# succinctlabs/sp1

Measured on AMD Instinct MI355X. Metric: RISC-V cycles proved/sec (core shard prove): whole ShardProof of a full core shard of the reference's `fibonacci` guest, see config, higher is better.
Workload: dtype u32 (KoalaBear Montgomery words, exact integer arithmetic)

## Files before the change

sp1_amd/csrc/basefold.hip:

```cpp
#include "device_ctx.hpp"
#include "tensor_table.hpp"

namespace sp1hip {

struct ExtArg { uint32_t c[4]; };
__device__ __forceinline__ kb::Ext E(const ExtArg& a) { return kb::Ext{{a.c[0], a.c[1], a.c[2], a.c[3]}}; }

__global__ __launch_bounds__(256) void transpose_kernel(const uint32_t* __restrict__ in, uint32_t* __restrict__ out,
                                                        size_t in_rows, size_t in_cols) {
    __shared__ uint32_t tile[32][33];
    const size_t r0 = (size_t)blockIdx.y * 32, c0 = (size_t)blockIdx.x * 32;
    const int tx = threadIdx.x & 31, ty = threadIdx.x >> 5;
    for (int k = ty; k < 32; k += 8) {
        size_t r = r0 + k, c = c0 + tx;
        if (r < in_rows && c < in_cols) tile[k][tx] = in[r * in_cols + c];
    }
    __syncthreads();
    for (int k = ty; k < 32; k += 8) {
        size_t c = c0 + k, r = r0 + tx;
        if (r < in_rows && c < in_cols) out[c * in_rows + r] = tile[tx][k];
    }
}

template <bool TO>
__global__ void monty_convert_kernel(uint32_t* data, size_t n) {
    size_t i = (size_t)blockIdx.x * blockDim.x + threadIdx.x;
    const size_t step = (size_t)gridDim.x * blockDim.x;
    for (; i < n; i += step) data[i] = TO ? kb::to_monty(data[i]) : kb::from_monty(data[i]);
}

__global__ __launch_bounds__(256) void batch_kernel(const uint32_t* const* __restrict__ cols, uint32_t total_width,
                                                    uint32_t height, const uint32_t* __restrict__ coeffs,
                                                    uint32_t* __restrict__ out) {
    const uint32_t row = blockIdx.x * 256u + threadIdx.x;
    if (row >= height) return;
    kb::DotAcc acc;
    kb::dot_init(acc);
    for (uint32_t g = 0; g < total_width; g++) {
        const kb::Ext c{{coeffs[4 * g], coeffs[4 * g + 1], coeffs[4 * g + 2], coeffs[4 * g + 3]}};
        kb::dot_add(acc, c, gptr(cols[g])[row]);
    }
    const kb::Ext r = kb::dot_finish(acc);
#pragma unroll
    for (int k = 0; k < 4; k++) out[(size_t)k * height + row] = r.c[k];
}

struct FoldOpenDesc {
    const uint32_t* cw;
    const uint32_t* tree;
    uint32_t lg_c, vals_off, paths_off, pad;
};

__device__ __forceinline__ void fold_even_odd_at(const uint32_t* __restrict__ cw, int lg_n, const ExtArg& half_beta,
                                                 const uint32_t* __restrict__ tw_lo, const uint32_t* __restrict__ tw_hi,
                                                 uint32_t* __restrict__ out, uint32_t i) {
    const uint32_t n = 1u << lg_n, m = n >> 1;
    kb::Ext e0, e1;
#pragma unroll
    for (int k = 0; k < 4; k++) {
        const uint2 v = *reinterpret_cast<const uint2*>(cw + (size_t)k * n + 2 * (size_t)i);
        e0.c[k] = v.x;
        e1.c[k] = v.y;
    }
    const uint32_t br = kb::reverse_bits_len(2 * i, lg_n);
    const uint32_t ex = ((n - br) & (n - 1)) << (kb::TWO_ADICITY - lg_n);
    const uint32_t xinv = kb::mul(tw_hi[ex >> TW_LO_BITS], tw_lo[ex & (TW_LO - 1)]);
    const uint32_t inv2 = 0x00ffffffu;
    kb::Ext s = kb::ext_mul_base(kb::ext_add(e0, e1), inv2);
    kb::Ext d = kb::ext_mul_base(kb::ext_sub(e0, e1), xinv);
    kb::Ext r = kb::ext_add(s, kb::ext_mul(d, E(half_beta)));
#pragma unroll
    for (int k = 0; k < 4; k++) out[(size_t)k * m + i] = r.c[k];
}
__global__ __launch_bounds__(256) void fold_even_odd_kernel(const uint32_t* __restrict__ cw, int lg_n, ExtArg half_beta,
                                                            const uint32_t* __restrict__ tw_lo,
                                                            const uint32_t* __restrict__ tw_hi,
                                                            uint32_t* __restrict__ out) {
    const uint32_t i = blockIdx.x * 256u + threadIdx.x;
    if (i < (1u << (lg_n - 1))) fold_even_odd_at(cw, lg_n, half_beta, tw_lo, tw_hi, out, i);
}

__device__ __forceinline__ kb::Ext fold_mle_at(const uint32_t* __restrict__ mle, int lg_n, const ExtArg& beta,
                                               uint32_t* __restrict__ out, uint32_t i) {
    const uint32_t n = 1u << lg_n, m = n >> 1;
    kb::Ext a, b;
#pragma unroll
    for (int k = 0; k < 4; k++) {
        const uint2 v = *reinterpret_cast<const uint2*>(mle + (size_t)k * n + 2 * (size_t)i);
        a.c[k] = v.x;
        b.c[k] = v.y;
    }
    kb::Ext r = kb::ext_add(a, kb::ext_mul(b, E(beta)));
#pragma unroll
    for (int k = 0; k < 4; k++) out[(size_t)k * m + i] = r.c[k];
    return r;
}
__global__ __launch_bounds__(256) void fold_mle_kernel(const uint32_t* __restrict__ mle, int lg_n, ExtArg beta,
                                                       uint32_t* __restrict__ out) {
    const uint32_t i = blockIdx.x * 256u + threadIdx.x;
    if (i < (1u << (lg_n - 1))) (void)fold_mle_at(mle, lg_n, beta, out, i);
}

__device__ __forceinline__ void block_sum4(uint32_t (&v)[4], uint32_t* scratch);

__global__ __launch_bounds__(256) void fold_round_kernel(const uint32_t* __restrict__ cw, int lg_c, ExtArg half_beta,
                                                         const uint32_t* __restrict__ tw_lo, const uint32_t* __restrict__ tw_hi,
                                                         uint32_t* __restrict__ cw_out, uint32_t cw_blocks,
                                                         const uint32_t* __restrict__ mle, int lg_m, ExtArg beta,
                                                         uint32_t* __restrict__ mle_out, const uint32_t* __restrict__ eq_next,
                                                         uint32_t* __restrict__ partial) {
    __shared__ uint32_t scratch[16];
    if (blockIdx.x < cw_blocks) {
        const uint32_t i = blockIdx.x * 256u + threadIdx.x;
        if (i < (1u << (lg_c - 1))) fold_even_odd_at(cw, lg_c, half_beta, tw_lo, tw_hi, cw_out, i);
        return;
    }
    const uint32_t b = blockIdx.x - cw_blocks, i = b * 256u + threadIdx.x, m = 1u << (lg_m - 1);
    kb::Ext term = kb::ext_zero();
    if (i < m) {
        const kb::Ext r = fold_mle_at(mle, lg_m, beta, mle_out, i);
        if (eq_next && !(i & 1u)) {
            const uint32_t j = i >> 1, half = m >> 1;
            kb::Ext e;
#pragma unroll
            for (int k = 0; k < 4; k++) e.c[k] = eq_next[(size_t)k * half + j];
            term = kb::ext_mul(e, r);
        }
// ... 269 lines not shown
    hipLaunchKernelGGL(fixed_at_zero_partial_kernel, dim3(blocks), dim3(256), 0, s, d_mle, n, d_eq, (uint32_t*)part.p);
    SP1HIP_LAUNCH_CHECK();
    launch_sum_partials((const uint32_t*)part.p, blocks, 4u, d_out, s);
    SP1HIP_LAUNCH_CHECK();
    return SP1HIP_SUCCESS;
}

int fold_round_async(const uint32_t* d_cw, int lg_c, const uint32_t* d_mle, int lg_m, const kb::Ext& beta, uint32_t* d_cw_out,
                     uint32_t* d_mle_out, const uint32_t* d_eq_next, uint32_t* d_zero_val, uint32_t* d_partial, hipStream_t s) {
    SP1HIP_REQUIRE(lg_c >= 1 && lg_c <= kb::TWO_ADICITY && lg_m >= 1 && lg_m <= 30, "fold sizes out of range");
    const DeviceCtx* ctx;
    SP1HIP_TRY(get_device_ctx(&ctx));
    ExtArg hb, b;
    for (int k = 0; k < 4; k++) { hb.c[k] = kb::mul(beta.c[k], 0x00ffffffu); b.c[k] = beta.c[k]; }
    const uint32_t cw_blocks = ((1u << (lg_c - 1)) + 255) / 256, mle_blocks = ((1u << (lg_m - 1)) + 255) / 256;
    hipLaunchKernelGGL(fold_round_kernel, dim3(cw_blocks + mle_blocks), dim3(256), 0, s, d_cw, lg_c, hb, ctx->d_tw_lo, ctx->d_tw_hi,
                       d_cw_out, cw_blocks, d_mle, lg_m, b, d_mle_out, d_eq_next, d_partial);
    SP1HIP_LAUNCH_CHECK();
    if (d_eq_next) {
        launch_sum_partials(d_partial, mle_blocks, 4u, d_zero_val, s);
        SP1HIP_LAUNCH_CHECK();
    }
    return SP1HIP_SUCCESS;
}

int eq_prefix_tables_soa_async(const kb::Ext* h_point, int d, uint32_t* d_out, hipStream_t s) {
    SP1HIP_REQUIRE(d >= 0 && d <= kb::TWO_ADICITY + 6, "dim out of range");
    PointArg pt;
    for (int j = 0; j < d; j++)
        for (int k = 0; k < 4; k++) pt.c[j][k] = h_point[j].c[k];
    hipLaunchKernelGGL(eq_prefix_soa_kernel, dim3(((1u << d) + 255) / 256), dim3(256), 0, s, pt, d, d_out);
    SP1HIP_LAUNCH_CHECK();
    return SP1HIP_SUCCESS;
}
}

extern "C" {

int sp1hip_transpose_to_col_major(uint32_t* d_out, const uint32_t* d_in, size_t rows, size_t cols, sp1hip_stream_t stream) {
    if (rows == 0 || cols == 0) return SP1HIP_SUCCESS;
    SP1HIP_REQUIRE(d_out && d_in && d_out != d_in, "bad buffers");
    dim3 grid((unsigned)((cols + 31) / 32), (unsigned)((rows + 31) / 32));
    SP1HIP_REQUIRE(grid.y <= 65535u * 1024u, "too many rows");
    hipLaunchKernelGGL(transpose_kernel, grid, dim3(256), 0, S(stream), d_in, d_out, rows, cols);
    SP1HIP_LAUNCH_CHECK();
    return SP1HIP_SUCCESS;
}

int sp1hip_transpose_to_row_major(uint32_t* d_out, const uint32_t* d_in, size_t rows, size_t cols, sp1hip_stream_t stream) {
    if (rows == 0 || cols == 0) return SP1HIP_SUCCESS;
    SP1HIP_REQUIRE(d_out && d_in && d_out != d_in, "bad buffers");
    dim3 grid((unsigned)((rows + 31) / 32), (unsigned)((cols + 31) / 32));
    hipLaunchKernelGGL(transpose_kernel, grid, dim3(256), 0, S(stream), d_in, d_out, cols, rows);
    SP1HIP_LAUNCH_CHECK();
    return SP1HIP_SUCCESS;
}

static int monty_convert(uint32_t* d, size_t n, bool to, sp1hip_stream_t stream) {
    if (!n) return SP1HIP_SUCCESS;
    SP1HIP_REQUIRE(d, "null buffer");
    size_t blocks = (n + 255) / 256;
    if (blocks > 4096) blocks = 4096;
    if (to) hipLaunchKernelGGL(monty_convert_kernel<true>, dim3((unsigned)blocks), dim3(256), 0, S(stream), d, n);
    else hipLaunchKernelGGL(monty_convert_kernel<false>, dim3((unsigned)blocks), dim3(256), 0, S(stream), d, n);
    SP1HIP_LAUNCH_CHECK();
    return SP1HIP_SUCCESS;
}
int sp1hip_to_monty(uint32_t* d, size_t n, sp1hip_stream_t s) { return monty_convert(d, n, true, s); }
int sp1hip_from_monty(uint32_t* d, size_t n, sp1hip_stream_t s) { return monty_convert(d, n, false, s); }

int sp1hip_basefold_batch(const sp1hip_tensor_t* tensors, int n_tensors, int lg_height, const uint32_t* d_coeffs,
                          uint32_t* d_out, sp1hip_stream_t stream) {
    SP1HIP_REQUIRE(lg_height >= 0 && lg_height <= 30, "lg_height out of range");
    SP1HIP_REQUIRE(d_coeffs && d_out, "null buffer");
    TensorTable tab;
    uint32_t tw;
    SP1HIP_TRY(make_tensor_table(tensors, n_tensors, &tab, &tw));
    SP1HIP_REQUIRE(tw <= 65536, "more than 2^16 columns in one message (batch_kernel's unreduced accumulators hold 2^16 terms)");
    hipStream_t s = S(stream);
    const uint32_t height = 1u << lg_height;
    AsyncScratch cols;
    SP1HIP_TRY(cols.alloc((size_t)tw * sizeof(uint32_t*), s));
    SP1HIP_TRY(expand_columns_async(tab, tw, height, (const uint32_t**)cols.p, s));
    hipLaunchKernelGGL(batch_kernel, dim3((height + 255) / 256), dim3(256), 0, s, (const uint32_t* const*)cols.p, tw,
                       height, d_coeffs, d_out);
    SP1HIP_LAUNCH_CHECK();
    return SP1HIP_SUCCESS;
}

int sp1hip_fold_even_odd(const uint32_t* d_cw, int lg_n, sp1hip_ext_t beta, uint32_t* d_out, sp1hip_stream_t stream) {
    SP1HIP_REQUIRE(lg_n >= 1 && lg_n <= kb::TWO_ADICITY, "lg_n out of range");
    SP1HIP_REQUIRE(d_cw && d_out, "null buffer");
    const DeviceCtx* ctx;
    SP1HIP_TRY(get_device_ctx(&ctx));
    ExtArg hb;
    for (int k = 0; k < 4; k++) hb.c[k] = kb::mul(beta.c[k], 0x00ffffffu);
    const uint32_t m = 1u << (lg_n - 1);
    hipLaunchKernelGGL(fold_even_odd_kernel, dim3((m + 255) / 256), dim3(256), 0, S(stream), d_cw, lg_n, hb,
                       ctx->d_tw_lo, ctx->d_tw_hi, d_out);
    SP1HIP_LAUNCH_CHECK();
    return SP1HIP_SUCCESS;
}

int sp1hip_fold_mle(const uint32_t* d_mle, int lg_n, sp1hip_ext_t beta, uint32_t* d_out, sp1hip_stream_t stream) {
    SP1HIP_REQUIRE(lg_n >= 1 && lg_n <= 30, "lg_n out of range");
    SP1HIP_REQUIRE(d_mle && d_out, "null buffer");
    ExtArg b;
    for (int k = 0; k < 4; k++) b.c[k] = beta.c[k];
    const uint32_t m = 1u << (lg_n - 1);
    hipLaunchKernelGGL(fold_mle_kernel, dim3((m + 255) / 256), dim3(256), 0, S(stream), d_mle, lg_n, b, d_out);
    SP1HIP_LAUNCH_CHECK();
    return SP1HIP_SUCCESS;
}

int sp1hip_partial_lagrange(const sp1hip_ext_t* h_point, int dim, uint32_t* d_out, sp1hip_stream_t stream) {
    SP1HIP_REQUIRE(dim >= 0 && dim <= kb::TWO_ADICITY + 6, "dim out of range");
    SP1HIP_REQUIRE(d_out && (h_point || dim == 0), "null buffer");
    hipStream_t s = S(stream);
    PointArg pt;
    for (int j = 0; j < dim; j++)
        for (int k = 0; k < 4; k++) pt.c[j][k] = h_point[j].c[k];
    const int d_hi = dim / 2, d_lo = dim - d_hi;
    AsyncScratch small;
    SP1HIP_TRY(small.alloc((((size_t)1 << d_hi) + ((size_t)1 << d_lo)) * 16, s));
    uint32_t* hi = (uint32_t*)small.p;
    uint32_t* lo = hi + ((size_t)4 << d_hi);
    hipLaunchKernelGGL(eq_small_kernel, dim3(((1u << d_hi) + 255) / 256), dim3(256), 0, s, pt, 0, d_hi, hi);
    SP1HIP_LAUNCH_CHECK();
    hipLaunchKernelGGL(eq_small_kernel, dim3(((1u << d_lo) + 255) / 256), dim3(256), 0, s, pt, d_hi, d_lo, lo);
    SP1HIP_LAUNCH_CHECK();
    const uint32_t len = 1u << dim;
    hipLaunchKernelGGL(eq_outer_kernel, dim3((len + 255) / 256), dim3(256), 0, s, hi, lo, d_lo, len, d_out);
    SP1HIP_LAUNCH_CHECK();
    return SP1HIP_SUCCESS;
}

int sp1hip_mle_eval_columns(const sp1hip_tensor_t* tensors, int n_tensors, int lg_height, const uint32_t* d_eq,
                            uint32_t* d_evals, sp1hip_stream_t stream) {
    SP1HIP_REQUIRE(lg_height >= 0 && lg_height <= 30, "lg_height out of range");
    SP1HIP_REQUIRE(d_eq && d_evals, "null buffer");
    TensorTable tab;
    uint32_t tw;
    SP1HIP_TRY(make_tensor_table(tensors, n_tensors, &tab, &tw));
    if (tw == 0) return SP1HIP_SUCCESS;
    SP1HIP_REQUIRE(tw <= 65536, "more than 2^16 columns in one message (the unreduced accumulators hold 2^16 terms)");
    hipStream_t s = S(stream);
    const uint32_t height = 1u << lg_height;
    AsyncScratch cols, part;
    SP1HIP_TRY(cols.alloc((size_t)tw * sizeof(uint32_t*), s));
    SP1HIP_TRY(expand_columns_async(tab, tw, height, (const uint32_t**)cols.p, s));
    const uint32_t chunks = (height + EVAL_ROWS - 1) / EVAL_ROWS;
    SP1HIP_TRY(part.alloc((size_t)chunks * tw * 16, s));
    dim3 grid((tw + EVAL_COLS - 1) / EVAL_COLS, chunks);
    hipLaunchKernelGGL(eval_columns_partial_kernel, grid, dim3(256), 0, s, (const uint32_t* const*)cols.p, tw, height,
                       d_eq, (uint32_t*)part.p);
    SP1HIP_LAUNCH_CHECK();
    launch_sum_partials((const uint32_t*)part.p, chunks, tw * 4, d_evals, s);
    SP1HIP_LAUNCH_CHECK();
    return SP1HIP_SUCCESS;
}

int sp1hip_ext_fixed_at_zero(const uint32_t* d_mle, int lg_n, const uint32_t* d_eq, uint32_t* d_out,
                             sp1hip_stream_t stream) {
    SP1HIP_REQUIRE(lg_n >= 1 && lg_n <= 30, "lg_n out of range");
    SP1HIP_REQUIRE(d_mle && d_eq && d_out, "null buffer");
    return ext_fixed_at_zero_async(d_mle, lg_n, d_eq, d_out, S(stream));
}

// ... 2 lines not shown
```

sp1_amd/csrc/gkr.hip:

```cpp
#include <algorithm>
#include <array>
#include <chrono>
#include <cstring>
#include <memory>
#include <string>
#include <vector>

#include "device_ctx.hpp"
#include "host_par.hpp"

namespace sp1hip {
bool gkr_host_simd_available();
void gkr_host_round_sums(const uint32_t* tab, size_t stride, const uint32_t* eq, size_t eq_stride, size_t real_pairs, uint32_t out[6][4]);
void gkr_host_round_fold(const uint32_t* tab, uint32_t* out, size_t stride, size_t real_pairs, const uint32_t alpha[4]);
}
#include "round_sync.hpp"
#include "tensor_table.hpp"

namespace sp1hip {

void challenger_observe(sp1hip_challenger_t* ch, uint32_t x);
kb::Ext challenger_sample_ext(sp1hip_challenger_t* ch);
void challenger_restore(sp1hip_challenger_t* dst, const sp1hip_challenger_t* src);
void challenger_export(const sp1hip_challenger_t* ch, uint32_t* w34);
// ... 420 lines not shown
        out[6] = (j & 1u) == 0 ? a[2] : z; out[7] = (j & 1u) == 0 ? z : a[2];
        out[8] = j < 2 ? a[3] : z;
        out[9] = a[4];
    } else {
        out[0] = j == 0 ? a[0] : z; out[1] = j == 1 ? a[0] : z;
        out[2] = a[1];
        out[3] = a[2];
    }
}

struct FlatArgs { const uint16_t* index; uint32_t total_slots; };

template <int FV, int SV, bool FIRST, bool NBASE, bool FLAT>
__global__ __launch_bounds__(256) void gkr_pass(const PassDesc* __restrict__ descs, const Ext* __restrict__ eq_int,
                                                const Ext* __restrict__ T, const Ext* __restrict__ TL, Ext a0, Ext a1,
                                                uint32_t* __restrict__ partials, RoundSync rs, uint32_t seq, uint32_t K,
                                                uint32_t tile_size, FlatArgs fa) {
    static_assert(FV + SV > 0 && FV <= 2 && SV <= 2, "a pass folds and / or sums");
    constexpr int SVS = SV == 0 ? 1 : SV;
    GridAcc<SVS> g;
    grid_init<SVS>(g);
    const uint32_t j = threadIdx.x & ((1u << SV) - 1u);
    auto do_row = [&](const PassDesc& d, uint32_t ro, bool valid, const Ext& wi, bool use_wi) {
        const uint32_t rows_out = (d.rows_in + (1u << FV) - 1u) >> FV;
        Row row = padding_row();
        if (valid && ro < rows_out) {
            row = fold_row<FV, FIRST, NBASE>(d, ro, a0, a1);
            if (FV > 0) {
                const uint32_t rq = folded_pos(ro, rows_out);
                if (SV == 0 && rs.host_slot != nullptr) {
                    st_ext_host(d.dst[0], rq, row.n0); st_ext_host(d.dst[1], rq, row.d0); st_ext_host(d.dst[2], rq, row.n1); st_ext_host(d.dst[3], rq, row.d1);
                } else {
                    st_ext(d.dst[0], rq, row.n0); st_ext(d.dst[1], rq, row.d0); st_ext(d.dst[2], rq, row.n1); st_ext(d.dst[3], rq, row.d1);
                }
            }
        }
        if constexpr (SV > 0) {
            const uint32_t cells = (rows_out + (1u << SV) - 1u) >> SV;
            const uint32_t c = ro >> SV;
            Ext w = kb::ext_zero(), wl = kb::ext_zero();
            if (valid && c < cells) {
                w = ld_ext(T, c); wl = ld_ext(TL, c);
                if (use_wi) { w = kb::ext_mul(w, wi); wl = kb::ext_mul(wl, wi); }
            }
            grid_accumulate<SVS, FIRST && NBASE && FV == 0>(row, w, wl, j, g);
        }
    };
    Ext scale = kb::ext_one();
    if (FLAT) {
        const uint32_t p = blockIdx.x * 256 + threadIdx.x;
        const bool valid = p < fa.total_slots;
        const PassDesc d = descs[valid ? fa.index[p] : 0];
        const Ext wi = SV > 0 ? ld_ext(eq_int, d.eq_int_index) : kb::ext_one();
        do_row(d, p - d.tile0, valid, wi, true);
    } else {
        const PassDesc d = descs[find_desc(descs, K, blockIdx.x)];
        const uint32_t rows_out = (d.rows_in + (1u << FV) - 1u) >> FV;
        const uint32_t slots = ((rows_out + (1u << SV) - 1u) >> SV) << SV;
        const uint32_t k0 = (blockIdx.x - d.tile0) * tile_size, k1 = min(slots, k0 + tile_size);
        for (uint32_t base = k0; base < k1; base += 256) do_row(d, base + threadIdx.x, base + threadIdx.x < k1, scale, false);
        if (SV > 0) scale = ld_ext(eq_int, d.eq_int_index);
    }
    if constexpr (SV > 0) {
        Ext out[GridOut<SVS>::NS];
        grid_split<SVS>(g, j, scale, !FLAT, out);
        rs_finish<GridOut<SVS>::NS>(out, partials, blockIdx.x, gridDim.x, rs, seq);
    } else if (rs.host_slot != nullptr) {
        asm volatile("s_waitcnt vmcnt(0)" ::: "memory");
        __syncthreads();
        if (threadIdx.x == 0 && rs_ticket_is_last_acq_rel(rs.counter, blockIdx.x, gridDim.x)) rs_publish_seq(rs.host_slot, seq);
    }
}

struct OpenDesc { const uint32_t* cols; uint32_t rows, width, col0, out0; };
constexpr int OPEN_COLS = 4, OPEN_ROWS = 16384;
__global__ __launch_bounds__(256) void open_columns_kernel(const OpenDesc* __restrict__ descs, const uint32_t* __restrict__ eq,
                                                           uint32_t eq_len, uint32_t* __restrict__ partials, uint32_t total_cols) {
    const OpenDesc d = descs[blockIdx.x];
    const uint32_t r0 = blockIdx.y * OPEN_ROWS;
    if (r0 >= d.rows) return;
    kb::DotAcc acc[OPEN_COLS];
#pragma unroll
    for (int c = 0; c < OPEN_COLS; c++) kb::dot_init(acc[c]);
    for (uint32_t r = r0 + threadIdx.x; r < r0 + OPEN_ROWS && r < d.rows; r += 256) {
        const Ext e{{eq[r], eq[eq_len + r], eq[2 * (size_t)eq_len + r], eq[3 * (size_t)eq_len + r]}};
#pragma unroll
        for (int c = 0; c < OPEN_COLS; c++)
            if (d.col0 + c < d.width) kb::dot_add(acc[c], e, gptr(d.cols)[(size_t)(d.col0 + c) * d.rows + r]);
    }
    __shared__ uint32_t sm[4][4 * OPEN_COLS];
    const int lane = threadIdx.x & 63, wave = threadIdx.x >> 6;
#pragma unroll
    for (int c = 0; c < OPEN_COLS; c++) {
        const Ext v = kb::dot_finish(acc[c]);
#pragma unroll
        for (int k = 0; k < 4; k++) {
            const uint32_t w = wave_sum(v.c[k]);
            if (lane == 0) sm[wave][4 * c + k] = w;
        }
    }
    __syncthreads();
    if (threadIdx.x < 4 * OPEN_COLS) {
        const int c = threadIdx.x / 4;
        if (d.col0 + c < d.width) {
            uint32_t a = 0;
            for (int i = 0; i < 4; i++) a = kb::add(a, sm[i][threadIdx.x]);
            partials[((size_t)blockIdx.y * total_cols + d.out0 + c) * 4 + (threadIdx.x & 3)] = a;
        }
    }
}
__global__ __launch_bounds__(256) void open_sum_kernel(const uint32_t* __restrict__ partials, uint32_t n_chunks, uint32_t n_words, uint32_t* __restrict__ out) {
    __shared__ uint32_t sm[256];
    const uint32_t jl = threadIdx.x & 63u, cl = threadIdx.x >> 6, j = blockIdx.x * 64u + jl;
    uint32_t acc = 0;
    if (j < n_words)
        for (uint32_t c = cl; c < n_chunks; c += 4) acc = kb::add(acc, partials[(size_t)c * n_words + j]);
    sm[threadIdx.x] = acc;
    __syncthreads();
    if (cl == 0 && j < n_words) out[j] = kb::add(kb::add(sm[jl], sm[64 + jl]), kb::add(sm[128 + jl], sm[192 + jl]));
}

Ext operator+(const Ext& a, const Ext& b) { return kb::ext_add(a, b); }
Ext operator-(const Ext& a, const Ext& b) { return kb::ext_sub(a, b); }
Ext operator*(const Ext& a, const Ext& b) { return kb::ext_mul(a, b); }
Ext ext_c(uint32_t canonical) { return kb::ext_from_base(kb::to_monty(canonical)); }
int log2_ceil(uint64_t x) { int l = 0; while (((uint64_t)1 << l) < x) l++; return l; }

std::vector<Ext> partial_lagrange_host(const std::vector<Ext>& pt) {
    std::vector<Ext> ev{kb::ext_one()};
    for (const Ext& x : pt) {
        std::vector<Ext> nx(ev.size() * 2);
        for (size_t i = 0; i < ev.size(); i++) { const Ext pr = ev[i] * x; nx[2 * i] = ev[i] - pr; nx[2 * i + 1] = pr; }
        ev.swap(nx);
    }
    return ev;
}
Ext eval_mle_host(const std::vector<Ext>& vals, const std::vector<Ext>& pt) {
    const std::vector<Ext> eq = partial_lagrange_host(pt);
    Ext acc = kb::ext_zero();
    for (size_t i = 0; i < vals.size(); i++) acc = acc + eq[i] * vals[i];
    return acc;
}

using Poly4 = std::array<Ext, 4>;
Ext poly_eval(const Poly4& c, const Ext& x) { return ((c[3] * x + c[2]) * x + c[1]) * x + c[0]; }

Poly4 interpolate4(const Ext (&xs)[4], const Ext (&ys)[4]) {
    Poly4 res{kb::ext_zero(), kb::ext_zero(), kb::ext_zero(), kb::ext_zero()};
    Ext num[4][4], den[4];
    bool live[4];
    for (int i = 0; i < 4; i++) {
        live[i] = !kb::ext_eq(ys[i], kb::ext_zero());
        if (!live[i]) continue;
        den[i] = kb::ext_one();
        Ext cur[4] = {ys[i], kb::ext_zero(), kb::ext_zero(), kb::ext_zero()};
        int deg = 0;
        for (int j = 0; j < 4; j++) {
            if (j == i) continue;
            den[i] = den[i] * (xs[i] - xs[j]);
            Ext nxt[4] = {kb::ext_zero(), kb::ext_zero(), kb::ext_zero(), kb::ext_zero()};
            for (int k = 0; k <= deg; k++) { nxt[k + 1] = nxt[k + 1] + cur[k]; nxt[k] = nxt[k] - cur[k] * xs[j]; }
            deg++;
            for (int k = 0; k < 4; k++) cur[k] = nxt[k];
        }
        for (int k = 0; k < 4; k++) num[i][k] = cur[k];
    }
    Ext prefix[4], running = kb::ext_one();
    for (int i = 0; i < 4; i++) if (live[i]) { prefix[i] = running; running = running * den[i]; }
    Ext inv_all = kb::ext_inv(running);
    for (int i = 3; i >= 0; i--) {
        if (!live[i]) continue;
// ... 738 lines not shown
```

sp1_amd/csrc/jagged.hip:

```cpp
#include <cstring>
#include <memory>
#include <vector>

#include <algorithm>
#include <array>

#include "device_ctx.hpp"
#include "jagged_host.hpp"
#include "round_sync.hpp"
#include "stacked_data.hpp"
#include "tensor_table.hpp"

namespace sp1hip {

struct DeviceBuf : AsyncScratch {
    uint32_t* u32() const { return (uint32_t*)p; }
};

void challenger_observe(sp1hip_challenger_t* ch, uint32_t x);
kb::Ext challenger_sample_ext(sp1hip_challenger_t* ch);
void challenger_restore(sp1hip_challenger_t* dst, const sp1hip_challenger_t* src);

using Ext = kb::Ext;

// ... 933 lines not shown
        uint32_t g = T;
        for (uint32_t pfx : prefix) g |= pfx;
        rf = g ? __builtin_ctz(g) : 0;
        rf = std::min(rf, std::min(log_m - 2, max_log_row_count - 1));
        if (!factored_enabled) rf = 0;
        if (rf < 2) rf = 0;
    }
    bool j_materialised = rf == 0;
    if (rf == 0) {
        SP1HIP_TRY(tabs[1].alloc((size_t)std::max<uint32_t>(n1, 1) * 16, s));
        SP1HIP_TRY(tabs[3].alloc((size_t)std::max<uint32_t>((n1 + 1) / 2, 1) * 16, s));
    }
    DeviceBuf row_eq_lv[2], d_prefix_lv;
    const uint32_t* row_eq_cur = d_row_eq.u32();
    uint32_t row_len_cur = 1u << max_log_row_count;
    if (rf) {
        SP1HIP_TRY(row_eq_lv[0].alloc(((size_t)16) << (max_log_row_count - 1), s));
        SP1HIP_TRY(row_eq_lv[1].alloc(((size_t)16) << (max_log_row_count - 1), s));
        SP1HIP_TRY(d_prefix_lv.alloc(prefix.size() * 4 * (size_t)(rf + 1), s));
        std::vector<uint32_t> all_lv(prefix.size() * (size_t)(rf + 1));
        for (int lv = 0; lv <= rf; lv++)
            for (size_t c = 0; c < prefix.size(); c++) all_lv[(size_t)lv * prefix.size() + c] = prefix[c] >> lv;
        SP1HIP_TRY(sc.stage.upload(d_prefix_lv.p, all_lv.data(), all_lv.size() * 4));
    }
    auto level_J = [&](int lv, const Ext& a_prev, JgJ* out) -> int {
        uint32_t* dst = row_eq_lv[lv & 1].u32();
        hipLaunchKernelGGL(jg_fold_row_eq, dim3((row_len_cur / 2 + 255) / 256), dim3(256), 0, s, row_eq_cur, row_len_cur, a_prev, dst);
        SP1HIP_LAUNCH_CHECK();
        row_eq_cur = dst;
        row_len_cur >>= 1;
        uint32_t* d_pl = d_prefix_lv.u32() + (size_t)lv * prefix.size();
        *out = JgJ{d_pl, ncols, (const Ext*)d_col_eq.p, row_eq_cur, row_len_cur};
        return SP1HIP_SUCCESS;
    };
    std::vector<JgTab> tabs0;
    uint32_t n_tiles0 = 0, n_tiles1 = 0, n_tiles2 = 0;
    bool tables_mult4 = false;
    bool skip_level1 = false;
    std::vector<std::pair<uint64_t, uint64_t>> zero_tails;
    DeviceBuf d_tabs0, d_col_eq3;
    {
        uint32_t g = T;
        for (uint32_t pfx : prefix) g |= pfx;
        if ((g & 1u) == 0 && factored_enabled) {
            uint64_t seg_start = 0;
            uint32_t col = 0;
            for (int r = 0; r < n_rounds; r++) {
                const StackedCore* d = rounds[r];
                uint64_t off = 0;
                const size_t n_real = d->row_counts.size() - 2;
                for (size_t t = 0; t < d->row_counts.size(); t++) {
                    const uint32_t h = (uint32_t)d->row_counts[t], w = (uint32_t)d->column_counts[t];
                    if (t < n_real && h && w) {
                        for (uint32_t c_lo = 0; c_lo < w; c_lo += JG_COL_SLICE) {
                            const uint32_t wc = std::min(JG_COL_SLICE, w - c_lo);
                            const uint64_t o = off + (uint64_t)c_lo * h;
                            tabs0.push_back(JgTab{(const uint32_t*)d->d_dense + o, h, col + c_lo, wc, n_tiles0, (uint32_t)(seg_start + o), n_tiles1, n_tiles2});
                            n_tiles0 += (h / 2 + JG_TAB_PAIRS - 1) / JG_TAB_PAIRS;
                            n_tiles1 += ((h + 3) / 4 + JG_TAB_PAIRS - 1) / JG_TAB_PAIRS;
                            n_tiles2 += ((h + 7) / 8 + JG_TAB_PAIRS - 1) / JG_TAB_PAIRS;
                        }
                    }
                    if (t == n_real) zero_tails.push_back({seg_start + off, seg_start + d->padded});
                    off += (uint64_t)h * w;
                    col += w;
                }
                seg_start += d->padded;
            }
            if (!tabs0.empty()) {
                SP1HIP_TRY(upload(d_tabs0, tabs0.data(), tabs0.size() * sizeof(JgTab), s, sc.stage));
                tables_mult4 = (g & 3u) == 0;
                skip_level1 = (g & 7u) == 0 && rf >= 2 && log_m >= 4;
                std::vector<Ext> col_eq3(col_eq.size());
                for (size_t c = 0; c < col_eq.size(); c++)
                    for (int q = 0; q < 4; q++) col_eq3[c].c[q] = kb::add(kb::dbl(col_eq[c].c[q]), col_eq[c].c[q]);
                SP1HIP_TRY(upload(d_col_eq3, col_eq3.data(), col_eq3.size() * 16, s, sc.stage));
            }
        }
    }
    SP1HIP_TRY(tabs[0].alloc((size_t)std::max<uint32_t>(skip_level1 ? (T + 7) / 8 : n1, 1) * 16, s));
    SP1HIP_TRY(tabs[2].alloc((size_t)std::max<uint32_t>((n1 + 1) / 2, 1) * 16, s));
    uint32_t n_live = T;
    int cur = 0;
    jg_t[1] = std::chrono::steady_clock::now();
    const bool lookahead01 = skip_level1 && !tabs0.empty() && log_m >= 2 && env_flag("SP1HIP_JAGGED_LOOKAHEAD", true);
    for (int round = 0; round < log_m; round++) {
        uint32_t nb;
        if (round == 0 && lookahead01) {
            {
                ScopedTimer t("jagged_round0_sum", s);
                nb = Scratch::blocks_for((uint64_t)n_tiles1 * 256);
                hipLaunchKernelGGL(jg_round01_tables, dim3(nb), dim3(256), 0, s, (const JgTab*)d_tabs0.p, (uint32_t)tabs0.size(), n_tiles1, J,
                                   sc.tail());
                SP1HIP_LAUNCH_CHECK();
            }
            Ext S[8];
            SP1HIP_TRY(sc.finish8(S));
            const Ext y0 = S[0] + S[1], h0 = S[2] + S[3];
            poly = interpolate(y0, h0, claim - y0);
            sumcheck.polys.push_back(poly);
            alpha = observe_and_sample(ch, poly);
            alphas.push_back(alpha);
            claim = poly_eval(poly, alpha);
            {
                JgJ J1;
                SP1HIP_TRY(level_J(1, alpha, &J1));
            }
            const Ext a0 = alpha;
            const Ext c0 = S[0], c2 = (S[0] + S[4]) + (S[0] + S[4]) - S[2], c1 = S[4] - c0 - c2;
            const Ext d0 = S[5], d2 = S[7], d1 = S[6] - d0 - d2;
            const Ext y1 = c0 + (c1 + c2 * a0) * a0, h1 = d0 + (d1 + d2 * a0) * a0;
            poly = interpolate(y1, h1, claim - y1);
            sumcheck.polys.push_back(poly);
            alpha = observe_and_sample(ch, poly);
            alphas.push_back(alpha);
            claim = poly_eval(poly, alpha);
            n_live = (n_live + 1) / 2;
            cur = 0;
            round = 1;
            continue;
        }
        if (round == 0) {
            ScopedTimer t("jagged_round0_sum", s);
            if (!tabs0.empty()) {
                nb = Scratch::blocks_for((uint64_t)n_tiles0 * 256);
                hipLaunchKernelGGL(jg_round0_tables, dim3(nb), dim3(256), 0, s, (const JgTab*)d_tabs0.p, (uint32_t)tabs0.size(), n_tiles0, J,
                                   sc.tail());
            } else {
                nb = Scratch::blocks_for((T / 2 + JG_ITERS - 1) / JG_ITERS);
                hipLaunchKernelGGL(jg_round0_sum, dim3(nb), dim3(256), 0, s, segs, J, T / 2, sc.tail());
            }
        } else if (round == 1) {
            ScopedTimer t("jagged_fold0_sum", s);
            const uint32_t n_out = (n_live + 1) / 2;
            nb = Scratch::blocks_for(((n_out + 1) / 2 + JG_ITERS - 1) / JG_ITERS);
            if (rf) {
                JgJ J1;
                SP1HIP_TRY(level_J(1, alpha, &J1));
                if (skip_level1) {
                    nb = Scratch::blocks_for((uint64_t)n_tiles1 * 256);
                    hipLaunchKernelGGL((jg_fold_tables<1, false>), dim3(nb), dim3(256), 0, s, (const JgTab*)d_tabs0.p, (uint32_t)tabs0.size(),
                                       n_tiles1, J1, (const Ext*)d_col_eq3.p, alpha, alpha, (Ext*)nullptr, sc.tail());
                } else if (tables_mult4) {
                    for (auto& z : zero_tails)
                        if (z.second > z.first) SP1HIP_HIP(hipMemsetAsync((Ext*)tabs[0].p + z.first / 2, 0, (size_t)((z.second - z.first) / 2) * 16, s));
                    nb = Scratch::blocks_for((uint64_t)n_tiles1 * 256);
                    hipLaunchKernelGGL((jg_fold_tables<1, true>), dim3(nb), dim3(256), 0, s, (const JgTab*)d_tabs0.p, (uint32_t)tabs0.size(),
                                       n_tiles1, J1, (const Ext*)d_col_eq3.p, alpha, alpha, (Ext*)tabs[0].p, sc.tail());
                } else {
                    hipLaunchKernelGGL(jg_fold0_sum<false>, dim3(nb), dim3(256), 0, s, segs, J, alpha, n_out, (Ext*)tabs[0].p, (Ext*)nullptr,
                                       sc.tail());
                }
            } else {
                hipLaunchKernelGGL(jg_fold0_sum<true>, dim3(nb), dim3(256), 0, s, segs, J, alpha, n_out, (Ext*)tabs[0].p, (Ext*)tabs[1].p,
                                   sc.tail());
            }
            n_live = n_out;
            cur = 0;
        } else {
            ScopedTimer t("jagged_fold_sum", s);
            const uint32_t n_out = (n_live + 1) / 2;
            const int nxt = cur ^ 2;
            if (round == 2 && skip_level1) {
                JgJ Jl;
                SP1HIP_TRY(level_J(2, alpha, &Jl));
                for (auto& z : zero_tails)
                    if (z.second > z.first) SP1HIP_HIP(hipMemsetAsync((Ext*)tabs[nxt].p + z.first / 4, 0, (size_t)((z.second - z.first) / 4) * 16, s));
                nb = Scratch::blocks_for((uint64_t)n_tiles2 * 256);
                hipLaunchKernelGGL((jg_fold_tables<2, true>), dim3(nb), dim3(256), 0, s, (const JgTab*)d_tabs0.p, (uint32_t)tabs0.size(),
                                   n_tiles2, Jl, (const Ext*)d_col_eq3.p, alphas[0], alpha, (Ext*)tabs[nxt].p, sc.tail());
            } else if (round <= rf) {
                JgJ Jl;
                SP1HIP_TRY(level_J(round, alpha, &Jl));
                nb = Scratch::blocks_for(((n_out + 1) / 2 + JG_ITERS - 1) / JG_ITERS);
                hipLaunchKernelGGL(jg_foldf_sum, dim3(nb), dim3(256), 0, s, (const Ext*)tabs[cur].p, n_live, Jl, alpha, n_out,
                                   (Ext*)tabs[nxt].p, sc.tail());
            } else {
                nb = Scratch::blocks_for((n_out + 1) / 2);
                if (!j_materialised) {
                    const JgJ Jp{d_prefix_lv.u32() + (size_t)(round - 1) * prefix.size(), ncols, (const Ext*)d_col_eq.p, row_eq_cur, row_len_cur};
                    SP1HIP_TRY(tabs[cur + 1].alloc((size_t)std::max<uint32_t>((n_out + 1) / 2, 1) * 16, s));
                    SP1HIP_TRY(tabs[nxt + 1].alloc((size_t)std::max<uint32_t>(n_out, 1) * 16, s));
                    j_materialised = true;
                    hipLaunchKernelGGL(jg_fold_sum_fj, dim3(nb), dim3(256), 0, s, (const Ext*)tabs[cur].p, Jp, n_live, alpha, n_out,
                                       (Ext*)tabs[nxt].p, (Ext*)tabs[nxt + 1].p, sc.tail());
                } else {
                    hipLaunchKernelGGL(jg_fold_sum, dim3(nb), dim3(256), 0, s, (const Ext*)tabs[cur].p, (const Ext*)tabs[cur + 1].p, n_live,
                                       alpha, n_out, (Ext*)tabs[nxt].p, (Ext*)tabs[nxt + 1].p, sc.tail());
                }
            }
            n_live = n_out;
            cur = nxt;
        }
        SP1HIP_LAUNCH_CHECK();
        Ext y0, h4;
        SP1HIP_TRY(sc.finish(nb, &y0, &h4));
        poly = interpolate(y0, h4, claim - y0);
        sumcheck.polys.push_back(poly);
        alpha = observe_and_sample(ch, poly);
        alphas.push_back(alpha);
        claim = poly_eval(poly, alpha);
    }
    sumcheck.point.assign(alphas.rbegin(), alphas.rend());
    sumcheck.eval = claim;
    if (log_m == 0) {
        SP1HIP_REQUIRE(false, "degenerate dense area");
    } else if (log_m == 1) {
        uint32_t hq[2];
        SP1HIP_TRY(sc.mb.fetch(rounds[0]->d_dense, 2, hq));
        q_eval = kb::ext_from_base(hq[0]) + kb::ext_mul_base(alpha, kb::sub(hq[1], hq[0]));
    } else {
        Ext hq[2] = {kb::ext_zero(), kb::ext_zero()}, hj[2] = {kb::ext_zero(), kb::ext_zero()};
        SP1HIP_TRY(sc.mb.fetch(tabs[cur].p, (size_t)n_live * 4, hq));
        SP1HIP_TRY(sc.mb.fetch(tabs[cur + 1].p, (size_t)n_live * 4, hj));
        q_eval = hq[0] + alpha * (hq[1] - hq[0]);
        j_eval = hj[0] + alpha * (hj[1] - hj[0]);
    }
    (void)j_eval;
    const std::vector<Ext>& final_point = sumcheck.point;

    jg_t[2] = std::chrono::steady_clock::now();
    marks.next("jagged_eval");
    Sumcheck jagged_eval;
    SP1HIP_TRY(jagged_eval_prove(prefix, log_m, z_row, z_col, final_point, ch, sc, &jagged_eval));
    jg_t[3] = std::chrono::steady_clock::now();
    marks.next("stacked_basefold_open");

    for (int k = 0; k < 4; k++) ch.observe(q_eval.c[k]);
    const std::vector<Ext> stack_point(final_point.end() - lsh, final_point.end());
    DeviceBuf d_eq, d_evals;
    SP1HIP_TRY(d_eq.alloc(((size_t)16) << lsh, s));
    SP1HIP_TRY(sp1hip_partial_lagrange(reinterpret_cast<const sp1hip_ext_t*>(stack_point.data()), lsh, d_eq.u32(), stream));
    std::vector<std::vector<Ext>> batch_evals(n_rounds);
    std::vector<Ext> flat_claims;
    SP1HIP_TRY(d_evals.alloc((size_t)(*std::max_element(round_widths.begin(), round_widths.end())) * 16, s));
    for (int r = 0; r < n_rounds; r++) {
        const uint32_t w = round_widths[r];
        batch_evals[r].resize(w);
        ScopedTimer t("jagged_batch_evals", s);
        SP1HIP_TRY(sp1hip_mle_eval_columns(rounds[r]->batches.data(), (int)rounds[r]->batches.size(), lsh, d_eq.u32(), d_evals.u32(), stream));
        SP1HIP_TRY(sc.mb.fetch(d_evals.p, (size_t)w * 4, batch_evals[r].data()));
        flat_claims.insert(flat_claims.end(), batch_evals[r].begin(), batch_evals[r].end());
    }
    for (auto& e : flat_claims) for (int k = 0; k < 4; k++) ch.observe(e.c[k]);
    jg_t[4] = std::chrono::steady_clock::now();
    size_t bf_len = need;
    SP1HIP_TRY(be.open(reinterpret_cast<const sp1hip_ext_t*>(stack_point.data()), lsh,
                       reinterpret_cast<const sp1hip_ext_t*>(flat_claims.data()), flat_claims.size(), config, h_proof, &bf_len, stream));

    jg_t[5] = std::chrono::steady_clock::now();
    Bytes w;
    w.p = h_proof;
    w.cap = need;
    w.n = bf_len;
    w.u64(n_rounds);
    for (auto& ev : batch_evals) { w.u64(ev.size()); for (auto& e : ev) w.ext(e); w.u64(1); w.u64(ev.size()); }
    sumcheck.write(w);
    jagged_eval.write(w);
    w.u64(n_rounds);
    for (int r = 0; r < n_rounds; r++) {
        w.u64(rounds[r]->row_counts.size());
        for (size_t t = 0; t < rounds[r]->row_counts.size(); t++) { w.u64(rounds[r]->row_counts[t]); w.u64(rounds[r]->column_counts[t]); }
    }
    w.u64(n_rounds);
    for (int r = 0; r < n_rounds; r++) {
        uint8_t c[64];
        be.write_commitment(r, c);
        w.raw(c, be.commitment_bytes());
    }
    w.ext(q_eval);
    w.u64(max_log_row_count);
    w.u64(log_m);
    if (w.overflow || w.n != need) {
        set_error("internal error: jagged proof size %zu != expected %zu", w.n, need);
        return SP1HIP_ERROR_RUNTIME;
    }
    *proof_len = w.n;
    be.accept();
    if (jg_timing) {
        jg_t[6] = std::chrono::steady_clock::now();
        const auto ms = [&](int a, int b) { return std::chrono::duration<double, std::milli>(jg_t[b] - jg_t[a]).count(); };
        fprintf(stderr, "[sp1hip jagged] set-up %.3f ms | %d sumcheck rounds %.3f | jagged-eval %.3f | column evaluations %.3f | BaseFold %.3f | proof bytes %.3f\n",
                ms(0, 1), log_m, ms(1, 2), ms(2, 3), ms(3, 4), ms(4, 5), ms(5, 6));
    }
    return SP1HIP_SUCCESS;
}

namespace {
struct InnerJaggedBackend final : JaggedBackend {
    sp1hip_challenger_t* caller;
    sp1hip_challenger_t* work = nullptr;
    sp1hip_stacked_data_t* const* rounds;
    int n_rounds;
    InnerJaggedBackend(sp1hip_challenger_t* c, sp1hip_stacked_data_t* const* r, int n) : caller(c), rounds(r), n_rounds(n) {}
    ~InnerJaggedBackend() override { sp1hip_challenger_free(work); }
    const char* entry_point() const override { return "sp1hip_jagged_prove"; }
    int begin() override { return sp1hip_challenger_clone(caller, &work); }
    void observe(uint32_t monty) override { challenger_observe(work, monty); }
    Ext sample_ext() override { return challenger_sample_ext(work); }
    void accept() override { challenger_restore(caller, work); }
    size_t opening_size(int dim, const uint32_t* widths, int n, sp1hip_fri_config_t config) const override {
        return sp1hip_basefold_proof_size(dim, widths, n, config);
    }
    int open(const sp1hip_ext_t* h_point, int dim, const sp1hip_ext_t* h_claims, size_t n_claims, sp1hip_fri_config_t config,
             uint8_t* h_proof, size_t* len, sp1hip_stream_t stream) override {
        std::vector<sp1hip_basefold_data_t*> bf;
        for (int r = 0; r < n_rounds; r++) bf.push_back(rounds[r]->basefold);
        return sp1hip_basefold_prove(h_point, dim, bf.data(), n_rounds, h_claims, n_claims, config, work, h_proof, len, stream);
    }
    size_t commitment_bytes() const override { return 32; }
    void write_commitment(int round, uint8_t* dst) const override {
        for (int k = 0; k < 8; k++) { const uint32_t v = kb::from_monty(rounds[round]->commit[k]); memcpy(dst + 4 * k, &v, 4); }
    }
};
}
}

using namespace sp1hip;

extern "C" {

int sp1hip_jagged_prove(const sp1hip_ext_t* h_z_row, int max_log_row_count, sp1hip_stacked_data_t* const* rounds, int n_rounds,
                        const sp1hip_ext_t* h_claims, const size_t* claims_per_round, sp1hip_fri_config_t config,
                        sp1hip_challenger_t* challenger, uint8_t* h_proof, size_t* proof_len, sp1hip_stream_t stream) {
    SP1HIP_REQUIRE(rounds && n_rounds > 0 && n_rounds <= 8 && challenger, "bad argument");
// ... 7 lines not shown
```

Baseline: 98.94 million.

## Reuse jagged sumcheck level-lsh table for batch evals; vectorize batch and open kernels

During the jagged sumcheck, the folded q table at level lsh is now kept in a separate buffer, and the per-column stacked evaluations are read from it. This replaces recomputing them with partial_lagrange plus mle_eval_columns over every column. Separately, the basefold batch kernel and the GKR column-opening kernel gain 128-bit vectorized paths that process four rows per thread when alignment allows. The first change costs an extra device buffer and adds coupling between the sumcheck layout and the batch order. The vector paths raise register pressure and reduce the number of threads.

```diff
diff --git a/sp1_amd/csrc/basefold.hip b/sp1_amd/csrc/basefold.hip
--- a/sp1_amd/csrc/basefold.hip
+++ b/sp1_amd/csrc/basefold.hip
@@ -43,6 +43,32 @@
     const kb::Ext r = kb::dot_finish(acc);
 #pragma unroll
     for (int k = 0; k < 4; k++) out[(size_t)k * height + row] = r.c[k];
+}
+
+__global__ __launch_bounds__(256) void batch_rows4_kernel(const uint32_t* const* __restrict__ cols, uint32_t total_width,
+                                                          uint32_t height, const uint32_t* __restrict__ coeffs,
+                                                          uint32_t* __restrict__ out) {
+    const uint32_t q = blockIdx.x * 256u + threadIdx.x;
+    if (q >= height / 4) return;
+    kb::DotAcc acc[4];
+#pragma unroll
+    for (int j = 0; j < 4; j++) kb::dot_init(acc[j]);
+    for (uint32_t g = 0; g < total_width; g++) {
+        const kb::Ext c{{coeffs[4 * g], coeffs[4 * g + 1], coeffs[4 * g + 2], coeffs[4 * g + 3]}};
+        const q4_t v = gptr(reinterpret_cast<const q4_t*>(cols[g]))[q];
+        kb::dot_add(acc[0], c, v.x);
+        kb::dot_add(acc[1], c, v.y);
+        kb::dot_add(acc[2], c, v.z);
+        kb::dot_add(acc[3], c, v.w);
+    }
+    kb::Ext r[4];
+#pragma unroll
+    for (int j = 0; j < 4; j++) r[j] = kb::dot_finish(acc[j]);
+#pragma unroll
+    for (int k = 0; k < 4; k++) {
+        const q4_t o = {r[0].c[k], r[1].c[k], r[2].c[k], r[3].c[k]};
+        gptr(reinterpret_cast<q4_t*>(out + (size_t)k * height))[q] = o;
+    }
 }
 
 struct FoldOpenDesc {
@@ -478,8 +504,14 @@
     AsyncScratch cols;
     SP1HIP_TRY(cols.alloc((size_t)tw * sizeof(uint32_t*), s));
     SP1HIP_TRY(expand_columns_async(tab, tw, height, (const uint32_t**)cols.p, s));
-    hipLaunchKernelGGL(batch_kernel, dim3((height + 255) / 256), dim3(256), 0, s, (const uint32_t* const*)cols.p, tw,
-                       height, d_coeffs, d_out);
+    bool rows4 = height >= 4 && ((uintptr_t)d_out & 15u) == 0;
+    for (int t = 0; t < tab.n; t++) rows4 = rows4 && (tab.col_start[t + 1] == tab.col_start[t] || ((uintptr_t)tab.base[t] & 15u) == 0);
+    if (rows4)
+        hipLaunchKernelGGL(batch_rows4_kernel, dim3((height / 4 + 255) / 256), dim3(256), 0, s, (const uint32_t* const*)cols.p, tw,
+                           height, d_coeffs, d_out);
+    else
+        hipLaunchKernelGGL(batch_kernel, dim3((height + 255) / 256), dim3(256), 0, s, (const uint32_t* const*)cols.p, tw,
+                           height, d_coeffs, d_out);
     SP1HIP_LAUNCH_CHECK();
     return SP1HIP_SUCCESS;
 }
diff --git a/sp1_amd/csrc/gkr.hip b/sp1_amd/csrc/gkr.hip
--- a/sp1_amd/csrc/gkr.hip
+++ b/sp1_amd/csrc/gkr.hip
@@ -526,11 +526,30 @@
     kb::DotAcc acc[OPEN_COLS];
 #pragma unroll
     for (int c = 0; c < OPEN_COLS; c++) kb::dot_init(acc[c]);
-    for (uint32_t r = r0 + threadIdx.x; r < r0 + OPEN_ROWS && r < d.rows; r += 256) {
-        const Ext e{{eq[r], eq[eq_len + r], eq[2 * (size_t)eq_len + r], eq[3 * (size_t)eq_len + r]}};
-#pragma unroll
-        for (int c = 0; c < OPEN_COLS; c++)
-            if (d.col0 + c < d.width) kb::dot_add(acc[c], e, gptr(d.cols)[(size_t)(d.col0 + c) * d.rows + r]);
+    if ((d.rows & 3u) == 0 && ((uintptr_t)d.cols & 15u) == 0) {
+        for (uint32_t r = r0 + 4 * threadIdx.x; r < r0 + OPEN_ROWS && r < d.rows; r += 4 * 256) {
+            q4_t ev[4];
+#pragma unroll
+            for (int k = 0; k < 4; k++) ev[k] = gptr(reinterpret_cast<const q4_t*>(eq + (size_t)k * eq_len + r))[0];
+            const Ext e0{{ev[0].x, ev[1].x, ev[2].x, ev[3].x}}, e1{{ev[0].y, ev[1].y, ev[2].y, ev[3].y}};
+            const Ext e2{{ev[0].z, ev[1].z, ev[2].z, ev[3].z}}, e3{{ev[0].w, ev[1].w, ev[2].w, ev[3].w}};
+#pragma unroll
+            for (int c = 0; c < OPEN_COLS; c++)
+                if (d.col0 + c < d.width) {
+                    const q4_t v = gptr(reinterpret_cast<const q4_t*>(d.cols + (size_t)(d.col0 + c) * d.rows + r))[0];
+                    kb::dot_add(acc[c], e0, v.x);
+                    kb::dot_add(acc[c], e1, v.y);
+                    kb::dot_add(acc[c], e2, v.z);
+                    kb::dot_add(acc[c], e3, v.w);
+                }
+        }
+    } else {
+        for (uint32_t r = r0 + threadIdx.x; r < r0 + OPEN_ROWS && r < d.rows; r += 256) {
+            const Ext e{{eq[r], eq[eq_len + r], eq[2 * (size_t)eq_len + r], eq[3 * (size_t)eq_len + r]}};
+#pragma unroll
+            for (int c = 0; c < OPEN_COLS; c++)
+                if (d.col0 + c < d.width) kb::dot_add(acc[c], e, gptr(d.cols)[(size_t)(d.col0 + c) * d.rows + r]);
+        }
     }
     __shared__ uint32_t sm[4][4 * OPEN_COLS];
     const int lane = threadIdx.x & 63, wave = threadIdx.x >> 6;
diff --git a/sp1_amd/csrc/jagged.hip b/sp1_amd/csrc/jagged.hip
--- a/sp1_amd/csrc/jagged.hip
+++ b/sp1_amd/csrc/jagged.hip
@@ -1039,6 +1039,12 @@
     SP1HIP_TRY(tabs[2].alloc((size_t)std::max<uint32_t>((n1 + 1) / 2, 1) * 16, s));
     uint32_t n_live = T;
     int cur = 0;
+    const bool evals_from_hq = log_m == lsh + 1, evals_from_q_eval = log_m == lsh;
+    const bool keep_level = log_m > lsh + 1 && !(lsh == 1 && skip_level1);
+    DeviceBuf d_q_lsh;
+    if (keep_level) SP1HIP_TRY(d_q_lsh.alloc((size_t)(T >> lsh) * 16, s));
+    auto q_slot = [&](int level, int slot) -> Ext* { return keep_level && level == lsh ? (Ext*)d_q_lsh.p : (Ext*)tabs[slot].p; };
+    const Ext* q_cur = nullptr;
     jg_t[1] = std::chrono::steady_clock::now();
     const bool lookahead01 = skip_level1 && !tabs0.empty() && log_m >= 2 && env_flag("SP1HIP_JAGGED_LOOKAHEAD", true);
     for (int round = 0; round < log_m; round++) {
@@ -1090,6 +1096,7 @@
         } else if (round == 1) {
             ScopedTimer t("jagged_fold0_sum", s);
             const uint32_t n_out = (n_live + 1) / 2;
+            Ext* const q_out = q_slot(1, 0);
             nb = Scratch::blocks_for(((n_out + 1) / 2 + JG_ITERS - 1) / JG_ITERS);
             if (rf) {
                 JgJ J1;
@@ -1100,38 +1107,39 @@
                                        n_tiles1, J1, (const Ext*)d_col_eq3.p, alpha, alpha, (Ext*)nullptr, sc.tail());
                 } else if (tables_mult4) {
                     for (auto& z : zero_tails)
-                        if (z.second > z.first) SP1HIP_HIP(hipMemsetAsync((Ext*)tabs[0].p + z.first / 2, 0, (size_t)((z.second - z.first) / 2) * 16, s));
+                        if (z.second > z.first) SP1HIP_HIP(hipMemsetAsync(q_out + z.first / 2, 0, (size_t)((z.second - z.first) / 2) * 16, s));
                     nb = Scratch::blocks_for((uint64_t)n_tiles1 * 256);
                     hipLaunchKernelGGL((jg_fold_tables<1, true>), dim3(nb), dim3(256), 0, s, (const JgTab*)d_tabs0.p, (uint32_t)tabs0.size(),
-                                       n_tiles1, J1, (const Ext*)d_col_eq3.p, alpha, alpha, (Ext*)tabs[0].p, sc.tail());
+                                       n_tiles1, J1, (const Ext*)d_col_eq3.p, alpha, alpha, q_out, sc.tail());
                 } else {
-                    hipLaunchKernelGGL(jg_fold0_sum<false>, dim3(nb), dim3(256), 0, s, segs, J, alpha, n_out, (Ext*)tabs[0].p, (Ext*)nullptr,
+                    hipLaunchKernelGGL(jg_fold0_sum<false>, dim3(nb), dim3(256), 0, s, segs, J, alpha, n_out, q_out, (Ext*)nullptr,
                                        sc.tail());
                 }
             } else {
-                hipLaunchKernelGGL(jg_fold0_sum<true>, dim3(nb), dim3(256), 0, s, segs, J, alpha, n_out, (Ext*)tabs[0].p, (Ext*)tabs[1].p,
+                hipLaunchKernelGGL(jg_fold0_sum<true>, dim3(nb), dim3(256), 0, s, segs, J, alpha, n_out, q_out, (Ext*)tabs[1].p,
                                    sc.tail());
             }
             n_live = n_out;
             cur = 0;
+            q_cur = q_out;
         } else {
             ScopedTimer t("jagged_fold_sum", s);
             const uint32_t n_out = (n_live + 1) / 2;
             const int nxt = cur ^ 2;
+            Ext* const q_out = q_slot(round, nxt);
             if (round == 2 && skip_level1) {
                 JgJ Jl;
                 SP1HIP_TRY(level_J(2, alpha, &Jl));
                 for (auto& z : zero_tails)
-                    if (z.second > z.first) SP1HIP_HIP(hipMemsetAsync((Ext*)tabs[nxt].p + z.first / 4, 0, (size_t)((z.second - z.first) / 4) * 16, s));
+                    if (z.second > z.first) SP1HIP_HIP(hipMemsetAsync(q_out + z.first / 4, 0, (size_t)((z.second - z.first) / 4) * 16, s));
                 nb = Scratch::blocks_for((uint64_t)n_tiles2 * 256);
                 hipLaunchKernelGGL((jg_fold_tables<2, true>), dim3(nb), dim3(256), 0, s, (const JgTab*)d_tabs0.p, (uint32_t)tabs0.size(),
-                                   n_tiles2, Jl, (const Ext*)d_col_eq3.p, alphas[0], alpha, (Ext*)tabs[nxt].p, sc.tail());
+                                   n_tiles2, Jl, (const Ext*)d_col_eq3.p, alphas[0], alpha, q_out, sc.tail());
             } else if (round <= rf) {
                 JgJ Jl;
                 SP1HIP_TRY(level_J(round, alpha, &Jl));
                 nb = Scratch::blocks_for(((n_out + 1) / 2 + JG_ITERS - 1) / JG_ITERS);
-                hipLaunchKernelGGL(jg_foldf_sum, dim3(nb), dim3(256), 0, s, (const Ext*)tabs[cur].p, n_live, Jl, alpha, n_out,
-                                   (Ext*)tabs[nxt].p, sc.tail());
+                hipLaunchKernelGGL(jg_foldf_sum, dim3(nb), dim3(256), 0, s, q_cur, n_live, Jl, alpha, n_out, q_out, sc.tail());
             } else {
                 nb = Scratch::blocks_for((n_out + 1) / 2);
                 if (!j_materialised) {
@@ -1139,15 +1147,16 @@
                     SP1HIP_TRY(tabs[cur + 1].alloc((size_t)std::max<uint32_t>((n_out + 1) / 2, 1) * 16, s));
                     SP1HIP_TRY(tabs[nxt + 1].alloc((size_t)std::max<uint32_t>(n_out, 1) * 16, s));
                     j_materialised = true;
-                    hipLaunchKernelGGL(jg_fold_sum_fj, dim3(nb), dim3(256), 0, s, (const Ext*)tabs[cur].p, Jp, n_live, alpha, n_out,
-                                       (Ext*)tabs[nxt].p, (Ext*)tabs[nxt + 1].p, sc.tail());
+                    hipLaunchKernelGGL(jg_fold_sum_fj, dim3(nb), dim3(256), 0, s, q_cur, Jp, n_live, alpha, n_out, q_out,
+                                       (Ext*)tabs[nxt + 1].p, sc.tail());
                 } else {
-                    hipLaunchKernelGGL(jg_fold_sum, dim3(nb), dim3(256), 0, s, (const Ext*)tabs[cur].p, (const Ext*)tabs[cur + 1].p, n_live,
-                                       alpha, n_out, (Ext*)tabs[nxt].p, (Ext*)tabs[nxt + 1].p, sc.tail());
+                    hipLaunchKernelGGL(jg_fold_sum, dim3(nb), dim3(256), 0, s, q_cur, (const Ext*)tabs[cur + 1].p, n_live, alpha, n_out,
+                                       q_out, (Ext*)tabs[nxt + 1].p, sc.tail());
                 }
             }
             n_live = n_out;
             cur = nxt;
+            q_cur = q_out;
         }
         SP1HIP_LAUNCH_CHECK();
         Ext y0, h4;
@@ -1160,6 +1169,7 @@
     }
     sumcheck.point.assign(alphas.rbegin(), alphas.rend());
     sumcheck.eval = claim;
+    std::vector<Ext> level_evals;
     if (log_m == 0) {
         SP1HIP_REQUIRE(false, "degenerate dense area");
     } else if (log_m == 1) {
@@ -1168,11 +1178,13 @@
         q_eval = kb::ext_from_base(hq[0]) + kb::ext_mul_base(alpha, kb::sub(hq[1], hq[0]));
     } else {
         Ext hq[2] = {kb::ext_zero(), kb::ext_zero()}, hj[2] = {kb::ext_zero(), kb::ext_zero()};
-        SP1HIP_TRY(sc.mb.fetch(tabs[cur].p, (size_t)n_live * 4, hq));
+        SP1HIP_TRY(sc.mb.fetch(q_cur, (size_t)n_live * 4, hq));
         SP1HIP_TRY(sc.mb.fetch(tabs[cur + 1].p, (size_t)n_live * 4, hj));
         q_eval = hq[0] + alpha * (hq[1] - hq[0]);
         j_eval = hj[0] + alpha * (hj[1] - hj[0]);
-    }
+        if (evals_from_hq) level_evals.assign(hq, hq + 2);
+    }
+    if (evals_from_q_eval) level_evals.assign(1, q_eval);
     (void)j_eval;
     const std::vector<Ext>& final_point = sumcheck.point;
 
@@ -1185,19 +1197,33 @@
 
     for (int k = 0; k < 4; k++) ch.observe(q_eval.c[k]);
     const std::vector<Ext> stack_point(final_point.end() - lsh, final_point.end());
-    DeviceBuf d_eq, d_evals;
-    SP1HIP_TRY(d_eq.alloc(((size_t)16) << lsh, s));
-    SP1HIP_TRY(sp1hip_partial_lagrange(reinterpret_cast<const sp1hip_ext_t*>(stack_point.data()), lsh, d_eq.u32(), stream));
     std::vector<std::vector<Ext>> batch_evals(n_rounds);
     std::vector<Ext> flat_claims;
-    SP1HIP_TRY(d_evals.alloc((size_t)(*std::max_element(round_widths.begin(), round_widths.end())) * 16, s));
-    for (int r = 0; r < n_rounds; r++) {
-        const uint32_t w = round_widths[r];
-        batch_evals[r].resize(w);
-        ScopedTimer t("jagged_batch_evals", s);
-        SP1HIP_TRY(sp1hip_mle_eval_columns(rounds[r]->batches.data(), (int)rounds[r]->batches.size(), lsh, d_eq.u32(), d_evals.u32(), stream));
-        SP1HIP_TRY(sc.mb.fetch(d_evals.p, (size_t)w * 4, batch_evals[r].data()));
-        flat_claims.insert(flat_claims.end(), batch_evals[r].begin(), batch_evals[r].end());
+    if (keep_level) {
+        level_evals.resize(T >> lsh);
+        SP1HIP_TRY(sc.mb.fetch(d_q_lsh.p, (size_t)(T >> lsh) * 4, level_evals.data()));
+    }
+    if (!level_evals.empty()) {
+        SP1HIP_REQUIRE(level_evals.size() == (size_t)(T >> lsh), "internal: level-lsh table size");
+        size_t off = 0;
+        for (int r = 0; r < n_rounds; r++) {
+            batch_evals[r].assign(level_evals.begin() + off, level_evals.begin() + off + round_widths[r]);
+            off += round_widths[r];
+        }
+        flat_claims = level_evals;
+    } else {
+        DeviceBuf d_eq, d_evals;
+        SP1HIP_TRY(d_eq.alloc(((size_t)16) << lsh, s));
+        SP1HIP_TRY(sp1hip_partial_lagrange(reinterpret_cast<const sp1hip_ext_t*>(stack_point.data()), lsh, d_eq.u32(), stream));
+        SP1HIP_TRY(d_evals.alloc((size_t)(*std::max_element(round_widths.begin(), round_widths.end())) * 16, s));
+        for (int r = 0; r < n_rounds; r++) {
+            const uint32_t w = round_widths[r];
+            batch_evals[r].resize(w);
+            ScopedTimer t("jagged_batch_evals", s);
+            SP1HIP_TRY(sp1hip_mle_eval_columns(rounds[r]->batches.data(), (int)rounds[r]->batches.size(), lsh, d_eq.u32(), d_evals.u32(), stream));
+            SP1HIP_TRY(sc.mb.fetch(d_evals.p, (size_t)w * 4, batch_evals[r].data()));
+            flat_claims.insert(flat_claims.end(), batch_evals[r].begin(), batch_evals[r].end());
+        }
     }
     for (auto& e : flat_claims) for (int k = 0; k < 4; k++) ch.observe(e.c[k]);
     jg_t[4] = std::chrono::steady_clock::now();
```

Result: no change. 98.88 million, median of 2 (-0.1%).
